# ChenFengTsai/dreamerv3-torch

Hardware: AMD Instinct MI355X
Metric: imagination-steps/sec (higher is better)
Workload: dtype f32; 1 GPU; cfg2: dmc_vision 64x64x3 synthetic replay, RSSM deter=512 hidden=512 stoch=32x32, continuous actor (6), imag_gradient dynamics, batch 16 x seq 64 per GPU, horizon 15; one step = full Dreamer._train update (world model + actor + critic fwd/bwd, gradient all-reduce, 3x clip+Adam); global_batch=16, seq_len=64, horizon=15, parallelism=dp1

## Files before the change

dreamerv3-torch_amd/csrc/fusedops.hip:

```cpp
#include "dv3_common.h"

namespace dv3 {

typedef float f32x4 __attribute__((ext_vector_type(4)));
typedef float f32x4u __attribute__((ext_vector_type(4), aligned(4)));

struct OLParams {
  const int* idx;
  int S, D;
  const float* x2;
  long ldx2;
  int A2;
  const float* WT;
  long ldw;
  const float* base;
  long ldbase;
  float* pre;
  long ldpre;
  const float* gamma;
  const float* beta;
  float* y;
  long ldy;
  float* mean;
  float* rstd;
  long M;
  int N;
  int act;
  const float* smp_logit;
  const float* smp_noise;
  const unsigned long long* smp_rng;
  unsigned long long smp_off;
  float* smp_onehot;
  int* smp_idx;
  const int* smp_forced;
  unsigned int* smp_flips;
  float smp_unimix;
  int smp_mode;
  const float* nb_first;
  const float* nb_init;
  const int* nb_init_idx;
  float* nb_out;
  int* nb_idx_out;
};

template <int NV4, bool SMP = false, bool RT = false>
__global__ __launch_bounds__(SMP ? 1024 : 256) void onehot_linear_ln_vec_kernel(OLParams p) {
  __shared__ __attribute__((aligned(16))) float part[4][256 * NV4];
  __shared__ int sidx[64];
  const int wave = threadIdx.x >> 6, l = threadIdx.x & 63;
  const float inv_n = 1.f / (float)p.N;
  constexpr int MAXB = 8;
  for (long r = blockIdx.x; r < p.M; r += gridDim.x) {
    int my;
    if constexpr (SMP) {
      const int d = threadIdx.x & 31;
      unsigned long long seed = 0, offset = 0;
      if (!p.smp_mode && !p.smp_noise) {
        seed = p.smp_rng[0];
        offset = p.smp_rng[1] + p.smp_off;
      }
      const float m = p.nb_first[r];
      __syncthreads();
      for (int sg = threadIdx.x >> 5; sg < p.S; sg += 32) {
        const long gi = r * p.S + sg;
        const float lg = p.smp_logit[gi * 32 + d];
        float sm, ph;
        unimix_probs<32>(lg, true, 32, p.smp_unimix, sm, ph);
        float score = ph;
        if (!p.smp_mode) {
          float q;
          if (p.smp_noise) {
            q = p.smp_noise[gi * 32 + d];
          } else {
            uint32_t o4[4];
            const unsigned long long e = (unsigned long long)gi * 32 + d;
            Philox ph4(seed);
            ph4(offset + (e >> 2), 0x5eedULL, o4);
            q = fmaxf(-logf(u01(o4[e & 3])), 1e-30f);
          }
          score = ph / q;
        }
        float best = score;
        int bi = d;
#pragma unroll
        for (int o = 16; o > 0; o >>= 1) {
          const float ob = __shfl_xor(best, o, 64);
          const int oi = __shfl_xor(bi, o, 64);
          if (ob > best || (ob == best && oi < bi)) {
            best = ob;
            bi = oi;
          }
        }
        if (p.smp_forced) {
          const int f = p.smp_forced[gi];
          if (d == 0 && p.smp_flips && f != bi) atomicAdd(p.smp_flips, 1u);
          bi = f;
        }
        const float v = (d == bi) ? 1.f : 0.f;
        p.smp_onehot[gi * 32 + d] = v;
        p.nb_out[gi * 32 + d] = v * (1.f - m) + p.nb_init[sg * 32 + d] * m;
        if (d == 0) {
          if (p.smp_idx) p.smp_idx[gi] = bi;
          const int ni = (m != 0.f) ? p.nb_init_idx[sg] : bi;
          p.nb_idx_out[gi] = ni;
          sidx[sg] = ni;
        }
      }
      __syncthreads();
      my = (l < p.S) ? sidx[l] : 0;
    } else {
      my = (l < p.S) ? p.idx[r * p.S + l] : 0;
    }
    const bool worker = !SMP || wave < 4;
    f32x4 acc[NV4];
#pragma unroll
    for (int v = 0; v < NV4; ++v) acc[v] = (f32x4){0.f, 0.f, 0.f, 0.f};
    if (worker) {
    if (wave == 0 && p.base) {
#pragma unroll
      for (int v = 0; v < NV4; ++v) acc[v] = *reinterpret_cast<const f32x4u*>(p.base + r * p.ldbase + 4 * (l + 64 * v));
    }
    for (int s0 = wave; s0 < p.S; s0 += 4 * MAXB) {
      f32x4 t[MAXB][NV4];
#pragma unroll
      for (int u = 0; u < MAXB; ++u) {
        const int s = s0 + 4 * u;
        if (s < p.S) {
          const int id = __builtin_amdgcn_readlane(my, s);
          const float* w = p.WT + (long)(s * p.D + id) * p.ldw + 4 * l;
#pragma unroll
          for (int v = 0; v < NV4; ++v) t[u][v] = *reinterpret_cast<const f32x4u*>(w + 256 * v);
        } else {
#pragma unroll
          for (int v = 0; v < NV4; ++v) t[u][v] = (f32x4){0.f, 0.f, 0.f, 0.f};
        }
      }
#pragma unroll
      for (int u = 0; u < MAXB; ++u)
#pragma unroll
        for (int v = 0; v < NV4; ++v) acc[v] += t[u][v];
    }
    for (int a = wave; a < p.A2; a += 4) {
      const float xa = p.x2[r * p.ldx2 + a];
      const float* w = p.WT + (long)(p.S * p.D + a) * p.ldw + 4 * l;
#pragma unroll
      for (int v = 0; v < NV4; ++v) acc[v] += xa * *reinterpret_cast<const f32x4u*>(w + 256 * v);
    }
    }
    __syncthreads();
    if (worker) {
#pragma unroll
      for (int v = 0; v < NV4; ++v) *reinterpret_cast<f32x4*>(&part[wave][4 * (l + 64 * v)]) = acc[v];
    }
    __syncthreads();
    if (!worker) continue;
#pragma unroll
    for (int v = 0; v < NV4; ++v) {
      const f32x4 a0 = *reinterpret_cast<const f32x4*>(&part[0][4 * (l + 64 * v)]);
      const f32x4 a1 = *reinterpret_cast<const f32x4*>(&part[1][4 * (l + 64 * v)]);
      const f32x4 a2 = *reinterpret_cast<const f32x4*>(&part[2][4 * (l + 64 * v)]);
      const f32x4 a3 = *reinterpret_cast<const f32x4*>(&part[3][4 * (l + 64 * v)]);
      acc[v] = (a0 + a1) + (a2 + a3);
      if ((v & 3) == wave) *reinterpret_cast<f32x4u*>(p.pre + r * p.ldpre + 4 * (l + 64 * v)) = acc[v];
    }
    if (!p.y) continue;
    float s = 0.f;
#pragma unroll
    for (int v = 0; v < NV4; ++v) s += (acc[v][0] + acc[v][1]) + (acc[v][2] + acc[v][3]);
    const float mean = group_sum<64>(s) * inv_n;
    float q = 0.f;
#pragma unroll
    for (int v = 0; v < NV4; ++v)
#pragma unroll
      for (int e = 0; e < 4; ++e) {
        const float d = acc[v][e] - mean;
        q += d * d;
      }
    const float rstd = rsqrtf(group_sum<64>(q) * inv_n + kLnEps);
#pragma unroll
    for (int v = 0; v < NV4; ++v) {
      if ((v & 3) != wave) continue;
      const f32x4 g = *reinterpret_cast<const f32x4u*>(p.gamma + 4 * (l + 64 * v));
      const f32x4 b = *reinterpret_cast<const f32x4u*>(p.beta + 4 * (l + 64 * v));
      f32x4 z;
#pragma unroll
      for (int e = 0; e < 4; ++e) {
        const float t = (acc[v][e] - mean) * rstd * g[e] + b[e];
        if constexpr (RT) z[e] = actf_(t, p.act);
        else z[e] = p.act ? siluf_(t) : t;
      }
      *reinterpret_cast<f32x4u*>(p.y + r * p.ldy + 4 * (l + 64 * v)) = z;
    }
    if (threadIdx.x == 0) {
      if (p.mean) p.mean[r] = mean;
      if (p.rstd) p.rstd[r] = rstd;
    }
  }
}

template <bool RT = false>
__global__ __launch_bounds__(256) void onehot_linear_ln_generic_kernel(OLParams p) {
  __shared__ float red[4];
  __shared__ int sidx[64];
  const int tid = threadIdx.x;
// ... 175 lines not shown
        } else {
          uint32_t o[4];
          Philox ph(seed);
          ph(offset + ((unsigned long long)e >> 2), 0x6e6f726dULL, o);
          const int j = (int)(e & 3);
          const float rad = sqrtf(-2.f * logf(u01(o[j & 2])));
          const float ang = 6.283185307179586f * u01(o[(j & 2) + 1]);
          eps = (j & 1) ? rad * sinf(ang) : rad * cosf(ang);
        }
        if (p.eps_out) p.eps_out[e] = eps;
        const float mu = tanhf(mr);
        const float sd = (p.max_std - p.min_std) * sigmoidf_(sr + 2.f) + p.min_std;
        const float pre = mu + sd * eps;
        p.action[e] = pre * (1.f / fmaxf(fabsf(pre), 1.f));
        en = 0.5f + 0.9189385332046727f + logf(sd);
      }
      en = group_sum<64>(en);
      if (l == 0 && p.ent) p.ent[r] = en;
    } else {
      const float m = group_max<64>(valid ? mr : -INFINITY);
      const float ex = valid ? expf(mr - m) : 0.f;
      const float sm = ex / group_sum<64>(ex);
      const float ph = valid ? sm * (1.f - p.unimix) + p.unimix / (float)p.A : 0.f;
      float qv = 1.f;
      if (valid) {
        if (p.noise) {
          qv = p.noise[e];
        } else {
          uint32_t o[4];
          Philox ph4(seed);
          ph4(offset + ((unsigned long long)e >> 2), 0x5eedULL, o);
          qv = fmaxf(-logf(u01(o[e & 3])), 1e-30f);
        }
      }
      float best = valid ? ph / qv : -INFINITY;
      int bi = l;
#pragma unroll
      for (int o = 32; o > 0; o >>= 1) {
        const float ob = __shfl_xor(best, o, 64);
        const int oi = __shfl_xor(bi, o, 64);
        if (ob > best || (ob == best && oi < bi)) {
          best = ob;
          bi = oi;
        }
      }
      if (p.forced) {
        const int f = p.forced[r];
        if (l == 0 && p.flips && f != bi) atomicAdd(p.flips, 1u);
        bi = f;
      }
      if (valid) p.action[e] = (l == bi) ? 1.f : 0.f;
      if (l == 0 && p.act_idx) p.act_idx[r] = bi;
      const float en = group_sum<64>(valid ? -ph * logf(ph) : 0.f);
      if (l == 0 && p.ent) p.ent[r] = en;
    }
  }
}

__global__ __launch_bounds__(256) void transpose2d_kernel(const float* __restrict__ src, long lds_, int R, int C,
                                                          float* __restrict__ dst, long ldd) {
  __shared__ float tile[32][33];
  const int tx = threadIdx.x & 31, ty = threadIdx.x >> 5;
  const int c0 = blockIdx.x * 32, r0 = blockIdx.y * 32;
#pragma unroll
  for (int j = 0; j < 32; j += 8) {
    const int r = r0 + ty + j, c = c0 + tx;
    tile[ty + j][tx] = (r < R && c < C) ? src[(long)r * lds_ + c] : 0.f;
  }
  __syncthreads();
#pragma unroll
  for (int j = 0; j < 32; j += 8) {
    const int c = c0 + ty + j, r = r0 + tx;
    if (c < C && r < R) dst[(long)c * ldd + r] = tile[tx][ty + j];
  }
}

constexpr int kTrJobs = 12;
struct TrJobs {
  const float* src[kTrJobs];
  float* dst[kTrJobs];
  long lds[kTrJobs], ldd[kTrJobs];
  int R[kTrJobs], C[kTrJobs], tiles_c[kTrJobs];
  int tile0[kTrJobs + 1];
  int n;
};
__global__ __launch_bounds__(256) void transpose2d_many_kernel(TrJobs jb) {
  __shared__ float tile[32][33];
  int k = 0;
  while (k + 1 < jb.n && (int)blockIdx.x >= jb.tile0[k + 1]) ++k;
  const int t = blockIdx.x - jb.tile0[k];
  const float* __restrict__ src = jb.src[k];
  float* __restrict__ dst = jb.dst[k];
  const long lds_ = jb.lds[k], ldd = jb.ldd[k];
  const int R = jb.R[k], C = jb.C[k];
  const int tx = threadIdx.x & 31, ty = threadIdx.x >> 5;
  const int c0 = (t % jb.tiles_c[k]) * 32, r0 = (t / jb.tiles_c[k]) * 32;
#pragma unroll
  for (int j = 0; j < 32; j += 8) {
    const int r = r0 + ty + j, c = c0 + tx;
    tile[ty + j][tx] = (r < R && c < C) ? src[(long)r * lds_ + c] : 0.f;
  }
  __syncthreads();
#pragma unroll
  for (int j = 0; j < 32; j += 8) {
    const int c = c0 + ty + j, r = r0 + tx;
    if (c < C && r < R) dst[(long)c * ldd + r] = tile[tx][ty + j];
  }
}

template <int G>
__global__ __launch_bounds__(256) void onehot_to_idx_kernel(const float* __restrict__ x, int* __restrict__ idx, long R,
                                                            int D) {
  constexpr int GPB = 256 / G;
  const int sub = threadIdx.x / G, d = threadIdx.x % G;
  for (long g0 = (long)blockIdx.x * GPB; g0 < R; g0 += (long)gridDim.x * GPB) {
    const long g = g0 + sub;
    float best = (g < R && d < D) ? x[g * D + d] : -INFINITY;
    int bi = d;
#pragma unroll
    for (int o = G / 2; o > 0; o >>= 1) {
      const float ob = __shfl_xor(best, o, 64);
      const int oi = __shfl_xor(bi, o, 64);
      if (ob > best || (ob == best && oi < bi)) {
        best = ob;
        bi = oi;
      }
    }
    if (g < R && d == 0) idx[g] = bi;
  }
}

static unsigned cap_grid(long n, long per_block, long cap) {
  long b = (n + per_block - 1) / per_block;
  if (b > cap) b = cap;
  if (b < 1) b = 1;
  return (unsigned)b;
}

}

using namespace dv3;

extern "C" int dv3_onehot_linear_ln_fwd(const int* idx, int S, int D, const float* x2, long ldx2, int A2,
                                        const float* WT, long ldw, const float* base, long ldbase, float* pre,
                                        long ldpre, const float* gamma, const float* beta, float* y, long ldy,
                                        float* mean, float* rstd, long M, int N, int act, void* stream) {
  if (M <= 0) return 0;
  if (!idx || !WT || !pre || S <= 0 || S > 64 || D <= 0 || N <= 0 || A2 < 0 || (A2 > 0 && !x2) || ldw < N ||
      ldpre < N || (base && ldbase < N) || !dv3_act_ok(act))
    return DV3_ERR_ARG;
  if (y && (!gamma || !beta || ldy < N)) return DV3_ERR_ARG;
  OLParams p{idx, S, D, x2, ldx2, A2, WT, ldw, base, ldbase, pre, ldpre, gamma, beta, y, ldy, mean, rstd, M, N, act};
  hipStream_t s = (hipStream_t)stream;
  const bool vec = (N % 256 == 0) && N <= 1024 && (ldw % 4 == 0) && (ldpre % 4 == 0) && (!base || ldbase % 4 == 0) &&
                   (!y || ldy % 4 == 0);
  if (vec) {
    const dim3 grid(cap_grid(M, 1, 32768)), block(256);
    if (dv3_act_rt(act)) switch (N / 256) {
      case 1: hipLaunchKernelGGL((onehot_linear_ln_vec_kernel<1, false, true>), grid, block, 0, s, p); break;
      case 2: hipLaunchKernelGGL((onehot_linear_ln_vec_kernel<2, false, true>), grid, block, 0, s, p); break;
      case 3: hipLaunchKernelGGL((onehot_linear_ln_vec_kernel<3, false, true>), grid, block, 0, s, p); break;
      default: hipLaunchKernelGGL((onehot_linear_ln_vec_kernel<4, false, true>), grid, block, 0, s, p); break;
    }
    else switch (N / 256) {
      case 1: hipLaunchKernelGGL((onehot_linear_ln_vec_kernel<1>), grid, block, 0, s, p); break;
      case 2: hipLaunchKernelGGL((onehot_linear_ln_vec_kernel<2>), grid, block, 0, s, p); break;
      case 3: hipLaunchKernelGGL((onehot_linear_ln_vec_kernel<3>), grid, block, 0, s, p); break;
      default: hipLaunchKernelGGL((onehot_linear_ln_vec_kernel<4>), grid, block, 0, s, p); break;
    }
  } else if (dv3_act_rt(act)) {
    hipLaunchKernelGGL(onehot_linear_ln_generic_kernel<true>, dim3(cap_grid(M, 1, 16384)), dim3(256), 0, s, p);
  } else {
    hipLaunchKernelGGL(onehot_linear_ln_generic_kernel<false>, dim3(cap_grid(M, 1, 16384)), dim3(256), 0, s, p);
  }
  return (int)hipGetLastError();
}

extern "C" int dv3_onehot_sample_linear_ln_fwd(const float* logit, const float* noise,
                                               const unsigned long long* rng_state, unsigned long long rng_offset,
                                               float* onehot, int* idx, const int* forced, unsigned int* flips,
                                               float unimix, int mode, const float* next_first, const float* init,
                                               const int* init_idx, float* next_out, int* next_idx, int S,
                                               const float* x2, long ldx2, int A2, const float* WT, long ldw,
                                               float* pre, long ldpre, const float* gamma, const float* beta, float* y,
                                               long ldy, float* mean, float* rstd, long M, int N, int act,
                                               void* stream) {
  if (M <= 0) return 0;
  if (!logit || !onehot || !next_first || !init || !init_idx || !next_out || !next_idx || !WT || !pre || !gamma ||
      !beta || !y || S <= 0 || S > 32 || N <= 0 || (N % 256) != 0 || N > 1024 || A2 < 0 || (A2 > 0 && !x2) ||
      ldw < N || ldpre < N || ldy < N || (ldw % 4) || (ldpre % 4) || (ldy % 4))
    return DV3_ERR_ARG;
  if (!dv3_act_ok(act) || dv3_act_rt(act)) return DV3_ERR_ARG;
  if (!mode && !noise && !rng_state) return DV3_ERR_ARG;
  OLParams p{nullptr, S, 32, x2, ldx2, A2, WT, ldw, nullptr, 0, pre, ldpre, gamma, beta, y, ldy, mean, rstd, M, N, act,
             logit, noise, rng_state, rng_offset, onehot, idx, forced, flips, unimix, mode, next_first, init, init_idx,
             next_out, next_idx};
  hipStream_t s = (hipStream_t)stream;
  const dim3 grid(cap_grid(M, 1, 32768)), block(1024);
  switch (N / 256) {
    case 1: hipLaunchKernelGGL((onehot_linear_ln_vec_kernel<1, true>), grid, block, 0, s, p); break;
    case 2: hipLaunchKernelGGL((onehot_linear_ln_vec_kernel<2, true>), grid, block, 0, s, p); break;
    case 3: hipLaunchKernelGGL((onehot_linear_ln_vec_kernel<3, true>), grid, block, 0, s, p); break;
    default: hipLaunchKernelGGL((onehot_linear_ln_vec_kernel<4, true>), grid, block, 0, s, p); break;
  }
  return (int)hipGetLastError();
}

extern "C" int dv3_actor_head_fwd_ex(const float* pre, long ldpre, const float* gamma, const float* beta, float* y,
                                     long ldy, float* mean, float* rstd, const float* Wm, const float* bm,
                                     const float* Ws, const float* bs, float* out_m, float* out_s, const float* noise,
                                     const unsigned long long* rng_state, unsigned long long rng_offset, float* eps_out,
                                     float* action, float* entropy, int* act_idx, const int* forced,
                                     unsigned int* flips, long M, int U, int A, float min_std, float max_std,
                                     float unimix, int onehot, int act, void* stream) {
  if (!dv3_act_ok(act)) return DV3_ERR_ARG;
  if (M <= 0) return 0;
  if (!pre || !gamma || !beta || !y || !Wm || !bm || !out_m || !action || U <= 0 || U > 1024 || A <= 0 || A > 64 ||
      ldpre < U || ldy < U)
    return DV3_ERR_ARG;
  if (!onehot && (!Ws || !bs || !out_s)) return DV3_ERR_ARG;
  if (onehot && Ws) return DV3_ERR_ARG;
  if (!noise && !rng_state) return DV3_ERR_ARG;
  AHParams p{pre, ldpre, gamma, beta, y, ldy, mean, rstd, Wm, bm, Ws, bs, out_m, out_s, noise, rng_state, rng_offset,
             eps_out, action, entropy, act_idx, forced, flips, M, U, A, min_std, max_std, unimix, onehot, act};
  hipStream_t s = (hipStream_t)stream;
  const dim3 grid(cap_grid(M, 4, 4096)), block(256);
  if (act != DV3_ACT_SILU) {
    if (U <= 64) hipLaunchKernelGGL((actor_head_kernel<1, true>), grid, block, 0, s, p);
    else if (U <= 256) hipLaunchKernelGGL((actor_head_kernel<4, true>), grid, block, 0, s, p);
    else if (U <= 512) hipLaunchKernelGGL((actor_head_kernel<8, true>), grid, block, 0, s, p);
    else hipLaunchKernelGGL((actor_head_kernel<16, true>), grid, block, 0, s, p);
    return (int)hipGetLastError();
  }
  if (U <= 64) hipLaunchKernelGGL((actor_head_kernel<1>), grid, block, 0, s, p);
  else if (U <= 256) hipLaunchKernelGGL((actor_head_kernel<4>), grid, block, 0, s, p);
  else if (U <= 512) hipLaunchKernelGGL((actor_head_kernel<8>), grid, block, 0, s, p);
  else hipLaunchKernelGGL((actor_head_kernel<16>), grid, block, 0, s, p);
  return (int)hipGetLastError();
}

extern "C" int dv3_actor_head_fwd(const float* pre, long ldpre, const float* gamma, const float* beta, float* y,
                                  long ldy, float* mean, float* rstd, const float* Wm, const float* bm,
                                  const float* Ws, const float* bs, float* out_m, float* out_s, const float* noise,
                                  const unsigned long long* rng_state, unsigned long long rng_offset, float* eps_out,
                                  float* action, float* entropy, int* act_idx, const int* forced,
                                  unsigned int* flips, long M, int U, int A, float min_std, float max_std,
                                  float unimix, int onehot, void* stream) {
  return dv3_actor_head_fwd_ex(pre, ldpre, gamma, beta, y, ldy, mean, rstd, Wm, bm, Ws, bs, out_m, out_s, noise, rng_state,
                               rng_offset, eps_out, action, entropy, act_idx, forced, flips, M, U, A, min_std, max_std,
                               unimix, onehot, DV3_ACT_SILU, stream);
}

extern "C" int dv3_transpose2d(const float* src, long lds, int R, int C, float* dst, long ldd, void* stream) {
  if (R <= 0 || C <= 0) return 0;
  if (!src || !dst || lds < C || ldd < R) return DV3_ERR_ARG;
  hipLaunchKernelGGL(transpose2d_kernel, dim3((C + 31) / 32, (R + 31) / 32), dim3(256), 0, (hipStream_t)stream, src,
                     lds, R, C, dst, ldd);
  return (int)hipGetLastError();
}

extern "C" int dv3_transpose2d_many(int njobs, const unsigned long long* jobs_host, void* stream) {
  if (njobs <= 0) return 0;
  if (!jobs_host || njobs > kTrJobs) return DV3_ERR_ARG;
  TrJobs jb;
  int tiles = 0;
  for (int k = 0; k < njobs; ++k) {
    const unsigned long long* j = jobs_host + 6 * k;
    jb.src[k] = (const float*)(uintptr_t)j[0];
    jb.dst[k] = (float*)(uintptr_t)j[1];
    jb.lds[k] = (long)j[2];
    jb.ldd[k] = (long)j[3];
    jb.R[k] = (int)j[4];
    jb.C[k] = (int)j[5];
    if (!jb.src[k] || !jb.dst[k] || jb.R[k] <= 0 || jb.C[k] <= 0 || jb.lds[k] < jb.C[k] || jb.ldd[k] < jb.R[k]) return DV3_ERR_ARG;
    jb.tiles_c[k] = (jb.C[k] + 31) / 32;
    jb.tile0[k] = tiles;
    tiles += jb.tiles_c[k] * ((jb.R[k] + 31) / 32);
  }
  for (int k = njobs; k <= kTrJobs; ++k) jb.tile0[k] = tiles;
  jb.n = njobs;
  hipLaunchKernelGGL(transpose2d_many_kernel, dim3((unsigned)tiles), dim3(256), 0, (hipStream_t)stream, jb);
  return (int)hipGetLastError();
}

extern "C" int dv3_onehot_to_idx(const float* onehot, int* idx, long R, int D, void* stream) {
  if (R <= 0) return 0;
  if (!onehot || !idx || D <= 0) return DV3_ERR_ARG;
  if (D > 64) return DV3_ERR_ARG;
  int G = 4;
  while (G < 64 && G < D) G <<= 1;
  hipStream_t s = (hipStream_t)stream;
  switch (G) {
    case 4: hipLaunchKernelGGL((onehot_to_idx_kernel<4>), dim3(cap_grid(R, 64, 8192)), dim3(256), 0, s, onehot, idx, R, D); break;
    case 8: hipLaunchKernelGGL((onehot_to_idx_kernel<8>), dim3(cap_grid(R, 32, 8192)), dim3(256), 0, s, onehot, idx, R, D); break;
    case 16: hipLaunchKernelGGL((onehot_to_idx_kernel<16>), dim3(cap_grid(R, 16, 8192)), dim3(256), 0, s, onehot, idx, R, D); break;
    case 32: hipLaunchKernelGGL((onehot_to_idx_kernel<32>), dim3(cap_grid(R, 8, 8192)), dim3(256), 0, s, onehot, idx, R, D); break;
    default: hipLaunchKernelGGL((onehot_to_idx_kernel<64>), dim3(cap_grid(R, 4, 8192)), dim3(256), 0, s, onehot, idx, R, D); break;
  }
  return (int)hipGetLastError();
}
```

dreamerv3-torch_amd/dv3hip/engine.py:

```python
from __future__ import annotations

from dataclasses import dataclass
from typing import Dict, List, Optional

import torch

from . import _dev, ops

F32 = torch.float32


_FUSE_BLEND = _dev.flag("DV3_FUSE_BLEND", True)
_FUSE_SAMPLE = _dev.flag("DV3_FUSE_SAMPLE", True)
_GATHER_OBS = _dev.flag("DV3_GATHER_OBS", True)
_FUSE_SAMPLE_IN = _dev.flag("DV3_FUSE_SAMPLE_IN", True)
_FUSE_CARRY = _dev.flag("DV3_FUSE_CARRY", True)
_FUSE_SCAN_ROW = _dev.flag("DV3_FUSE_SCAN_ROW", True)
_FUSE_SCAN_LN = _dev.flag("DV3_FUSE_SCAN_LN", True)
_FUSE_SCAN_LNBWD = _dev.flag("DV3_FUSE_SCAN_LNBWD", True)
_FUSE_SCAN_CS = _dev.flag("DV3_FUSE_SCAN_CS", True)
_DEFER_CONV_WGRAD = _dev.flag("DV3_DEFER_CONV_WGRAD", True)
_FUSE_SCAN_GRUBWD = _dev.flag("DV3_FUSE_SCAN_GRUBWD", True)
_ONEHOT_WGRAD = _dev.flag("DV3_ONEHOT_WGRAD", True)
_ONEHOT_WGRAD_MIN_WORK = 1 << 21
# ... 926 lines not shown
                               eps_out=bufs["eps"], mode=not sample, **self.head)
            return
        io = None if idx_out is None else idx_out.view(-1)
        if fuse_smp:
            ops.gemm_sample(bufs["x2"], P.ims.W, bufs["logit"].view(M, self.SD), bufs["stoch"], bias=P.ims.b,
                            noise=noise, rng=rng, idx=io, forced=forced, flips=flips, unimix=self.unimix,
                            mode=not sample)
        else:
            ops.gemm(bufs["x2"], P.ims.W, bufs["logit"].view(M, self.SD), bias=P.ims.b)
            ops.onehot_sample(bufs["logit"], bufs["stoch"], noise=noise, rng=rng, unimix=self.unimix, mode=not sample,
                              forced=forced, flips=flips, idx=io)

    def pack_bwd(self, defer=None):
        P, ws = self.P, self.ws
        wt = {"in": self.pack_img_in(defer=defer)}
        for nm, W in (("gru", P.gru.W), ("out", P.img_out.W), ("ims", P.ims.W)):
            t = ws.get(f"rssm.{nm}_wt", (W.shape[1], W.shape[0]))
            if defer is not None:
                defer.append((W, t))
            else:
                ops.transpose2d(W, t)
            wt[nm] = t
        return wt

    def img_step_bwd(self, dstoch, ddeter, prev_deter, bufs, scratch, dprev_stoch, dprev_deter, daction,
                     accumulate_prev=False, wt=None):
        P = self.P
        M = dstoch.shape[0]
        S, D, SD, De, Hd = self.S, self.D, self.SD, self.De, self.Hd
        dlogit = scratch["dlogit"]
        if self.gauss:
            ops.gauss_head_bwd(bufs["raw"], dlogit, dstoch=dstoch, eps=bufs["eps"], **self.head_bwd)
        else:
            ops.onehot_st_bwd(bufs["logit"], dstoch.view(M, S, D), dlogit.view(M, S, D), unimix=self.unimix)
        if wt is not None:
            ops.gemm(dlogit, wt["ims"], scratch["dx2"])
            dense_ln_bwd_pre(P.img_out, scratch["dx2"], bufs["x2pre"], bufs.get("m2"), bufs.get("r2"), scratch["dx2pre"],
                             wgrad=False)
            ops.gemm(scratch["dx2pre"], wt["out"], ddeter, accumulate=True)
            gru_gates_bwd(P.gru, ddeter, bufs["gpre"], prev_deter, bufs.get("mg"), bufs.get("rg"), scratch["dgpre"],
                          dprev_deter, wgrad=False, accumulate_dh=accumulate_prev)
            if M > 128 and ops.gemm_split_ok(scratch["dgpre"], wt["gru"]):
                ops.gemm_split(scratch["dgpre"], wt["gru"], scratch["dx1"], dprev_deter, accumulate2=True)
            else:
                ops.gemm(scratch["dgpre"], wt["gru"][Hd:], dprev_deter, accumulate=True)
                ops.gemm(scratch["dgpre"], wt["gru"][:Hd], scratch["dx1"])
            dense_ln_bwd_pre(P.img_in, scratch["dx1"], bufs["x1pre"], bufs.get("m1"), bufs.get("r1"), scratch["dx1pre"],
                             wgrad=False)
            if daction is not None and M > 128 and SD % 16 == 0 and ops.gemm_split_ok(scratch["dx1pre"], wt["in"]):
                ops.gemm_split(scratch["dx1pre"], wt["in"], dprev_stoch, daction, accumulate=accumulate_prev)
                return
            ops.gemm(scratch["dx1pre"], wt["in"][:SD], dprev_stoch, accumulate=accumulate_prev)
            if daction is not None:
                ops.gemm(scratch["dx1pre"], wt["in"][SD:], daction)
            return
        ops.gemm(dlogit, P.ims.W, scratch["dx2"], transB=False)
        dense_ln_bwd_pre(P.img_out, scratch["dx2"], bufs["x2pre"], bufs.get("m2"), bufs.get("r2"), scratch["dx2pre"],
                         wgrad=False)
        ops.gemm(scratch["dx2pre"], P.img_out.W, ddeter, transB=False, accumulate=True)
        gru_gates_bwd(P.gru, ddeter, bufs["gpre"], prev_deter, bufs.get("mg"), bufs.get("rg"), scratch["dgpre"],
                      dprev_deter, wgrad=False, accumulate_dh=accumulate_prev)
        ops.gemm(scratch["dgpre"], P.gru.W[:, Hd:], dprev_deter, transB=False, accumulate=True)
        ops.gemm(scratch["dgpre"], P.gru.W[:, :Hd], scratch["dx1"], transB=False)
        dense_ln_bwd_pre(P.img_in, scratch["dx1"], bufs["x1pre"], bufs.get("m1"), bufs.get("r1"), scratch["dx1pre"],
                         wgrad=False)
        ops.gemm(scratch["dx1pre"], P.img_in.W[:, :SD], dprev_stoch, transB=False, accumulate=accumulate_prev)
        if daction is not None:
            ops.gemm(scratch["dx1pre"], P.img_in.W[:, SD:], daction, transB=False)


@dataclass
class PConvLayer:
    W: torch.Tensor
    g: Optional[torch.Tensor] = None
    b: Optional[torch.Tensor] = None
    bias: Optional[torch.Tensor] = None
    act: int = 1
    out: bool = False

    def __post_init__(self):
        if self.bias is not None:
            self.out = True


_IM2COL_ROWS = _dev.value("DV3_IM2COL_ROWS", 2048)


class ConvEncoderEngine:
    def __init__(self, layers: List[PConvLayer], ws: Workspace, size=64):
        self.L, self.ws, self.size = layers, ws, size

    def forward(self, image_u8=None, perm=None, x_f32=None, keep=True):
        ws = self.ws
        H = self.size
        if x_f32 is not None:
            x, N = x_f32, x_f32.shape[0]
        else:
            N = image_u8.shape[0] * image_u8.shape[1]
            C = image_u8.shape[-1]
            x = ws.get("enc.x0", (N, H, H, C))
            ops.image_to_f32(image_u8, x, n_images=N, perm=perm)
        self._acts = []
        n_layers = len(self.L)
        for i, L in enumerate(self.L):
            Co, Ci = L.W.shape[0], L.W.shape[1]
            OH = H // 2
            pre = ws.get(f"enc.pre{i}", (N, OH, OH, Co))
            if N * OH * OH <= _IM2COL_ROWS and not keep:
                cols = ws.get(f"enc.cols{i}", (N * OH * OH, 16 * Ci))
                ops.im2col_s2(x, cols)
                ops.gemm(cols, L.W.view(Co, 16 * Ci), pre.view(N * OH * OH, Co))
            elif Ci == 3 and Co in ops.C3_WIDTHS:
                ops.conv_s2_c3_fwd(x, L.W, pre, CW=Co)
            else:
                wp = ws.get(f"enc.wp{i}", (Co, 16 * Ci))
                ops.pack_conv_weight(L.W, wp, transposed=False)
                ops.conv_s2_fwd(x, wp, pre, Ci=Ci, Co=Co)
            R = N * OH * OH
            mean, rstd = (ws.get(f"enc.m{i}", (R,)), ws.get(f"enc.r{i}", (R,))) if L.g is not None else (None, None)
            last = i == n_layers - 1
            y = ws.get(f"enc.y{i}", (N, Co * OH * OH) if last else (N, OH, OH, Co))
            ln_fwd(L, pre.view(R, Co), y if last else y.view(R, Co), mean, rstd, chw_group=OH * OH if last else 0)
            self._acts.append((x, pre, mean, rstd, y))
            x, H = y, OH
        return x

    def backward(self, dembed):
        ws = self.ws
        n_layers = len(self.L)
        dy = dembed
        for i in reversed(range(n_layers)):
            L = self.L[i]
            x, pre, mean, rstd, y = self._acts[i]
            Co, Ci = L.W.shape[0], L.W.shape[1]
            N, OH = pre.shape[0], pre.shape[1]
            R = N * OH * OH
            last = i == n_layers - 1
            dpre = ws.get(f"enc.dpre{i}", pre.shape)
            ln_bwd(L, dy if last else dy.view(R, Co), pre.view(R, Co), mean, rstd, dpre.view(R, Co), wgrad=True,
                   chw_group=OH * OH if last else 0)
            ops.conv_s2_wgrad(dpre, x, _g(L.W))
            if i > 0:
                wpt = ws.get(f"enc.wpt{i}", (4, Ci, 4 * Co))
                ops.pack_conv_weight(L.W, wpt, transposed=True)
                dx = ws.get(f"enc.dy{i - 1}", x.shape)
                ops.convT_s2_fwd(dpre, wpt, dx, Ci=Co, Co=Ci)
                dy = dx


class ConvDecoderEngine:
    def __init__(self, lin: PLin, layers: List[PConvLayer], ws: Workspace, minres=4):
        self.lin, self.L, self.ws, self.minres = lin, layers, ws, minres

    def forward(self, x1, x2):
        ws = self.ws
        R = x1.shape[0]
        E = self.lin.W.shape[0]
        mr = self.minres
        C0 = E // (mr * mr)
        h0 = ws.get("dec.h0", (R, mr, mr, C0))
        ops.gemm(x1, self.lin.W, h0.view(R, E), A2=x2, bias=self.lin.b)
        self._x = (x1, x2)
        self._acts = []
        x, H = h0, mr
        for i, L in enumerate(self.L):
            Ci, Co = L.W.shape[0], L.W.shape[1]
            OH = 2 * H
            c3 = L.out and Co == 3 and Ci in ops.C3_WIDTHS
            if not c3:
                wpt = ws.get(f"dec.wpt{i}", (4, Co, 4 * Ci))
                ops.pack_conv_weight(L.W, wpt, transposed=True)
            if not L.out:
                pre = ws.get(f"dec.pre{i}", (R, OH, OH, Co))
                ops.convT_s2_fwd(x, wpt, pre, Ci=Ci, Co=Co)
                rows = R * OH * OH
                mean, rstd = (ws.get(f"dec.m{i}", (rows,)), ws.get(f"dec.r{i}", (rows,))) if L.g is not None \
                    else (None, None)
                y = ws.get(f"dec.y{i}", (R, OH, OH, Co))
                ln_fwd(L, pre.view(rows, Co), y.view(rows, Co), mean, rstd)
                self._acts.append((x, pre, mean, rstd, y))
            else:
                y = ws.get("dec.recon", (R, OH, OH, Co))
                if c3:
                    ops.convT_s2_c3_fwd(x, L.W, y, CW=Ci, bias=L.bias, out_add=0.5)
                else:
                    ops.convT_s2_fwd(x, wpt, y, Ci=Ci, Co=Co, bias=L.bias, out_add=0.5)
                self._acts.append((x, None, None, None, y))
            x, H = y, OH
        return x

    def backward(self, drecon, dx1, dx2, *, acc_dx=False, defer=None, idx=None, D=0):
        ws = self.ws
        run = defer.append if defer is not None else (lambda f: f())
        dy = drecon
        for i in reversed(range(len(self.L))):
            L = self.L[i]
            x, pre, mean, rstd, y = self._acts[i]
            Ci, Co = L.W.shape[0], L.W.shape[1]
            R, OH = y.shape[0], y.shape[1]
            rows = R * OH * OH
            if not L.out:
                dpre = ws.get(f"dec.dpre{i}", pre.shape)
                ln_bwd(L, dy.view(rows, Co), pre.view(rows, Co), mean, rstd, dpre.view(rows, Co), wgrad=True)
            else:
                dpre = dy
                if L.bias is not None:
                    run(lambda dpre=dpre, L=L, rows=rows, Co=Co: ops.colsum(dpre.view(rows, Co), _g(L.bias),
                                                                         accumulate=True))
            (run if _DEFER_CONV_WGRAD else (lambda f: f()))(lambda x=x, dpre=dpre, L=L: ops.conv_s2_wgrad(x, dpre, _g(L.W)))
            dx = ws.get(f"dec.dx{i}", x.shape)
            if Co == 3 and Ci in ops.C3_WIDTHS:
                ops.conv_s2_c3_fwd(dpre, L.W, dx, CW=Ci)
            else:
                wp = ws.get(f"dec.wp{i}", (Ci, 16 * Co))
                ops.pack_conv_weight(L.W, wp, transposed=False)
                ops.conv_s2_fwd(dpre, wp, dx, Ci=Co, Co=Ci)
            dy = dx
        R = dy.shape[0]
        E = self.lin.W.shape[0]
        dh0 = dy.view(R, E)
        x1, x2 = self._x

        def _lin_wg():
            lin_wgrad_onehot(ws, "dec.lin", self.lin.W, dh0, idx, D, x1, x2)
            ops.colsum(dh0, _g(self.lin.b), accumulate=True)

        run(_lin_wg)
        k1 = x1.shape[1]
        ops.gemm(dh0, self.lin.W[:, :k1], dx1, transB=False, accumulate=acc_dx)
        ops.gemm(dh0, self.lin.W[:, k1:], dx2, transB=False, accumulate=acc_dx)


class EnsembleEngine:

    def __init__(self, name: str, bucket, layers: int, ws: Workspace, *, std: float, scale: float = 1.0, log: bool = True,
                 act=True):
        if bucket.members < 2 or layers < 1:
            raise ValueError("EnsembleEngine: needs at least 2 members (the unbiased std) and 1 trunk layer")
        self.name, self.bucket, self.L, self.ws = name, bucket, int(layers), ws
        self.K = bucket.members
        self.std, self.scale, self.log = float(std), float(scale), bool(log)
        self.act = ops.act_code(act)
        self._kept = None
        self._loss_ws = torch.zeros(ops.ENS_LOSS_WS, dtype=F32, device=ws.device)

    def _params(self):
        st = self.bucket.stacked
        layers = [(st(3 * i), st(3 * i + 1), st(3 * i + 2)) for i in range(self.L)]
        return layers, st(3 * self.L), st(3 * self.L + 1)

    def _acts(self, M: int, tag: str):
        layers, _, _ = self._params()
        ws, nm, K = self.ws, f"{self.name}.{tag}", self.K
        acts = []
        for i, ((W, _), _, _) in enumerate(layers):
            U = W.shape[1]
            acts.append((ws.get(f"{nm}.pre{i}", (K, M, U)), ws.get(f"{nm}.m{i}", (K * M,)),
                         ws.get(f"{nm}.r{i}", (K * M,)), ws.get(f"{nm}.y{i}", (K, M, U))))
        return acts

    def _trunk_fwd(self, x, tag: str):
        layers, _, _ = self._params()
        acts = self._acts(x.shape[0], tag)
        h = x
        for ((W, _), (g, _), (b, _)), (pre, mean, rstd, y) in zip(layers, acts):
            ops.ens_gemm(h, W, pre)
            ops.ens_ln_act_fwd(pre, g, b, y, mean, rstd, act=self.act)
            h = y
        return h, acts

    def _trunk_bwd(self, x, acts, dh, tag: str, *, wgrad: bool, dx=None, cols=None):
        layers, _, _ = self._params()
        ws, nm, K, M = self.ws, f"{self.name}.{tag}", self.K, x.shape[0]
        dy = dh
        for i in reversed(range(self.L)):
            (W, gW), (g, gg), (b, gb) = layers[i]
            pre, mean, rstd, _ = acts[i]
            dpre = ws.get(f"{nm}.dpre{i}", tuple(pre.shape))
            ops.ens_ln_act_bwd(dy, pre, g, b, mean, rstd, dpre, gg if wgrad else None, gb if wgrad else None,
                               act=self.act)
            if wgrad:
                ops.ens_gemm(dpre, acts[i - 1][3] if i > 0 else x, gW, transA=True, transB=False, accumulate=True)
            if i > 0:
                dprev = ws.get(f"{nm}.dy{i - 1}", tuple(acts[i - 1][3].shape))
                ops.ens_gemm(dpre, W, dprev, transB=False)
                dy = dprev
            elif dx is not None:
                ops.ens_gemm(dpre, W if cols is None else W[:, :, cols], dx, transB=False)

    def forward(self, x):
        _, (Wh, _), (bh, _) = self._params()
        M = x.shape[0]
        h, _ = self._trunk_fwd(x, f"f{M}")
        mu = self.ws.get(f"{self.name}.f{M}.mu", (self.K, M, Wh.shape[1]))
        ops.ens_gemm(h, Wh, mu, bias=bh)
        ops.tanh_fwd(mu, mu)
        return mu

    def regress_fwd_bwd(self, x, target):
        _, (Wh, gWh), (bh, gbh) = self._params()
        M, ws, nm = x.shape[0], self.ws, f"{self.name}.t{x.shape[0]}"
        h, acts = self._trunk_fwd(x, f"t{M}")
        pre = ws.get(f"{nm}.out", (self.K, M, Wh.shape[1]))
        ops.ens_gemm(h, Wh, pre, bias=bh)
        loss = ws.get(f"{nm}.loss", (1,))
        ops.ens_regress_loss(pre, target, pre, loss, self._loss_ws, self.std)
        ops.ens_gemm(pre, h, gWh, transA=True, transB=False, accumulate=True)
        ops.ens_colsum(pre, gbh, accumulate=True)
        dh = ws.get(f"{nm}.dh", tuple(h.shape))
        ops.ens_gemm(pre, Wh, dh, transB=False)
        self._trunk_bwd(x, acts, dh, f"t{M}", wgrad=True)
        return loss.view(())

    def disag_fwd(self, x, reward=None, *, keep: bool = True):
# ... 30 lines not shown
```

dreamerv3-torch_amd/models.py:

```python
from __future__ import annotations

import copy

import numpy as np
import torch
from torch import nn

import networks
import tools
from dv3hip import _dev
from dv3hip import engine as E
from dv3hip import ops
from dv3hip.params import ParamBucket

to_np = lambda x: x.detach().cpu().numpy()
_FUSED_IMAG = _dev.flag("DV3_FUSED_IMAG", True)
_STACK_DETER = _dev.flag("DV3_STACK_DETER", True)


import weakref

_BEHAVIORS = weakref.WeakKeyDictionary()
_RUNNERS = weakref.WeakKeyDictionary()

# ... 74 lines not shown
            self.dynamics = networks.RSSM(config.dyn_stoch, config.dyn_deter, config.dyn_hidden, config.dyn_rec_depth,
                                          config.dyn_discrete, config.act, config.norm, config.dyn_mean_act,
                                          config.dyn_std_act, config.dyn_min_std, config.unimix_ratio, config.initial,
                                          config.num_actions, self.embed_size, config.device)
            self.heads = nn.ModuleDict()
            feat_size = config.dyn_stoch * (config.dyn_discrete or 1) + config.dyn_deter
            self.heads["decoder"] = networks.MultiDecoder(feat_size, shapes, **config.decoder)
            self.heads["reward"] = networks.MLP(
                feat_size, (255,) if config.reward_head["dist"] == "symlog_disc" else (), config.reward_head["layers"],
                config.units, config.act, config.norm, dist=config.reward_head["dist"],
                outscale=config.reward_head["outscale"], device=config.device, name="Reward")
            self.heads["cont"] = networks.MLP(
                feat_size, (), config.cont_head["layers"], config.units, config.act, config.norm, dist="binary",
                outscale=config.cont_head["outscale"], device=config.device, name="Cont")
        if config.reward_head["dist"] != "symlog_disc":
            raise NotImplementedError("reward head: symlog_disc only")
        for name in config.grad_heads:
            assert name in self.heads, name
        self._model_opt = tools.Optimizer("model", list(self.parameters()), config.model_lr, config.opt_eps,
                                          config.grad_clip, config.weight_decay, opt=config.opt, use_amp=False)
        self._scales = dict(reward=config.reward_head["loss_scale"], cont=config.cont_head["loss_scale"])

    def preprocess(self, obs):
        dev = self._config.device
        obs = {k: torch.as_tensor(np.asarray(v) if not isinstance(v, torch.Tensor) else v).to(dev).to(torch.float32)
               for k, v in obs.items()}
        obs["image"] = obs["image"] / 255.0
        if "discount" in obs:
            obs["discount"] = (obs["discount"] * self._config.discount).unsqueeze(-1)
        assert "is_first" in obs and "is_terminal" in obs
        obs["cont"] = (1.0 - obs["is_terminal"]).unsqueeze(-1)
        return obs

    def _stage(self, data):
        dev = torch.device(self._config.device)
        out = {}
        for k, v in data.items():
            if isinstance(v, torch.Tensor):
                t = v.to(dev, non_blocking=True)
            else:
                t = torch.from_numpy(np.ascontiguousarray(v)).to(dev, non_blocking=True)
            if k == "image":
                if t.dtype != torch.uint8:
                    t = torch.clamp(torch.round(t.to(torch.float32)), 0, 255).to(torch.uint8)
                out[k] = t.contiguous()
            else:
                out[k] = t.to(torch.float32).contiguous()
        return out

    @tools.on_config_device
    def _train(self, data, noise=None):
        r = self._auto_runner() if noise is None else None
        if r is None:
            return self._train_eager(data, noise)
        return r.train_wm(data)

    def _auto_runner(self):
        r = _RUNNERS.get(self)
        if r is None:
            cfg = self._config
            beh = next((b() for b in _BEHAVIORS.get(self, []) if b() is not None), None)
            if (beh is None or not bool(getattr(cfg, "hip_graph", True)) or not torch.cuda.is_available()
                    or torch.device(cfg.device).type != "cuda"):
                return None
            from dv3hip.graph import UpdateRunner

            r = UpdateRunner(self, beh, use_graph=True)
            _RUNNERS[self] = r
        return r

    def _train_eager(self, data, noise=None):
        self.train_fwd_bwd(data, noise)
        return self.train_opt()

    def train_opt(self, allreduce=True):
        post, context, metrics, loss = self._pending
        metrics = dict(metrics)
        metrics.update(self._model_opt.finish(loss, allreduce))
        return post, context, _wrap(metrics)

    def train_fwd_bwd(self, data, noise=None):
        cfg = self._config
        st = self._stage(data)
        B, T = st["action"].shape[0], st["action"].shape[1]
        TB = B * T
        dev = st["action"].device
        dyn = self.dynamics
        rssm = dyn.engine
        ws = rssm.ws
        S, D, SD, De = dyn._stoch, dyn._discrete, dyn._stoch * (dyn._discrete or 1), dyn._deter
        gauss = not D
        nz = noise or {}
        rng = dyn._rng()
        self._model_opt.begin()

        act_tm = ops.transpose01(st["action"], ws.get("wm.action", (T, B, st["action"].shape[2])))
        first_tm = ops.transpose01(st["is_first"], ws.get("wm.first", (T, B)))
        reward_tm = ops.transpose01(st["reward"], ws.get("wm.reward", (T, B)))
        cont_tm = ws.get("wm.cont", (T, B))
        ops.transpose01(st["is_terminal"], cont_tm)
        ops.axpby(ws.get("wm.ones", (T, B)).fill_(1.0), cont_tm, 1.0, -1.0)

        enc = self.encoder
        cnn_eng = mlp_eng = None
        parts = []
        if enc.cnn_shapes:
            cnn_eng = enc._cnn.engine
            parts.append(cnn_eng.forward(st["image"], (B, T)))
        if enc.mlp_shapes:
            keys = list(enc.mlp_shapes)
            widths = [int(np.prod(enc.mlp_shapes[k])) for k in keys]
            xin = ws.get("wm.mlp_in", (TB, sum(widths)))
            raw = ws.get("wm.mlp_raw", (TB, sum(widths)))
            off = 0
            for k, w in zip(keys, widths):
                tmp = ops.transpose01(st[k].reshape(B, T, w), ws.get(f"wm.key.{k}", (T, B, w)))
                raw[:, off:off + w] = tmp.view(TB, w)
                off += w
            ops.symlog(raw, xin)
            mlp_eng = enc._mlp.engine_for(".wm")
            parts.append(mlp_eng.forward(xin)[0])
            self._enc_in = xin
        if len(parts) == 2:
            Ec, Em = parts[0].shape[1], parts[1].shape[1]
            embed = ws.get("wm.embed", (TB, Ec + Em))
            embed[:, :Ec].copy_(parts[0])
            embed[:, Ec:].copy_(parts[1])
        else:
            embed = parts[0]
        E_ = embed.shape[1]

        force = None
        if "force_post" in nz or "force_prior" in nz:
            force = dict(post=nz.get("force_post"), prior=nz.get("force_prior"), flips=nz.get("flips"))
        out = rssm.observe_fwd(embed.view(T, B, E_), act_tm, first_tm, q_prior=nz.get("q_prior"),
                               q_post=nz.get("q_post"), rng=rng, force=force)
        ps, dt = out["post_stoch"].view(TB, SD), out["deter"].view(TB, De)
        kl = ws.get("wm.kl", (T, B))
        ent_p, ent_q = ws.get("wm.ent_post", (T, B)), ws.get("wm.ent_prior", (T, B))
        if gauss:
            ops.gauss_kl_fwd(out["post_mean"], out["post_std"], out["prior_mean"], out["prior_std"], kl, ent_p, ent_q)
        else:
            ops.kl_fwd(out["post_logit"], out["prior_logit"], kl, ent_p, ent_q, unimix=dyn._unimix_ratio)
        lanes_pay = rssm.lanes_pay(heavy_side=bool(self.heads["decoder"].cnn_shapes))
        E.SideStream.host_sync_point(lanes_pay)

        up = 1.0 / TB
        dec = self.heads["decoder"]
        acc = ws.zeros("wm.acc", (8 + len(dec.mlp_shapes),))
        gs, gd = ws.get("wm.gs", (T, B, SD)), ws.get("wm.gd", (T, B, De))
        wrote = False
        deferred = []
        grad_heads = cfg.grad_heads
        if dec.cnn_shapes:
            dec_eng = dec._cnn.engine
            recon = dec_eng.forward(ps, dt)
            limg = ws.get("wm.loss_img", (TB,))
            drecon = ws.get("wm.drecon", recon.shape)
            ops.mse_image(recon, st["image"], limg, drecon, upstream=up, perm=(B, T))
            ops.dot_accumulate(limg, acc[1:2], scale=up)
            dec_eng.backward(drecon, gs.view(TB, SD), gd.view(TB, De), acc_dx=False, defer=deferred,
                             idx=out["post_idx"].view(TB, S) if E._GATHER_OBS and not gauss else None, D=D)
            self._defer_heads_from = len(deferred)
            wrote = True
            if "decoder" not in grad_heads:
                gs.zero_(), gd.zero_()
        if dec.mlp_shapes:
            mdec = dec._mlp
            deng = mdec.engine_for(".wm")
            h, _, _ = deng.forward(ps, dt)
            dh = ws.zeros("wm.dec_dh", h.shape)
            for ki, (k, shp) in enumerate(dec.mlp_shapes.items()):
                lin = mdec.mean_layer[k]
                w = int(np.prod(shp))
                mode = ws.get(f"wm.dec.{k}", (TB, w))
                ops.gemm(h, lin.weight, mode, bias=lin.bias)
                tgt = ops.transpose01(st[k].reshape(B, T, w), ws.get(f"wm.key.{k}", (T, B, w))).view(TB, w)
                lk = ws.get(f"wm.loss.{k}", (TB,))
                dmode = ws.get(f"wm.dmode.{k}", (TB, w))
                ops.symlog_mse(mode, tgt, lk, dmode, upstream=up)
                ops.dot_accumulate(lk, acc[8 + ki:9 + ki], scale=up)
                ops.gemm(dmode, lin.weight, dh, transB=False, accumulate=True)
                E.lin_wgrad(lin.weight, dmode, h)
                ops.colsum(dmode, lin.bias.grad, accumulate=True)
            gh = "decoder" in grad_heads
            deng.backward(ps, dt, slice(0, TB), wgrad=True, dh=dh, dx1=gs.view(TB, SD) if gh else None,
                          dx2=gd.view(TB, De) if gh else None, acc_dx=wrote, defer=deferred)
            wrote = wrote or gh
        if not wrote:
            gs.zero_(), gd.zero_()
        pidx = out["post_idx"].view(TB, S) if E._GATHER_OBS and not gauss else None
        reng = self.heads["reward"].engine_for(".wm")
        if pidx is not None:
            reng.pack_onehot(SD)
        _, r_logits, _ = reng.forward(ps, dt, idx=pidx, D=D)
        lp_r = ws.get("wm.lp_r", (TB,))
        ops.disc_logprob_fwd(r_logits, reward_tm.view(TB), lp_r)
        ops.dot_accumulate(lp_r, acc[2:3], scale=-up)
        dr = ws.get("wm.dr_logits", r_logits.shape)
        up_r = ws.get("wm.up_r", (TB,)).fill_(-up * self._scales["reward"])
        ops.disc_logprob_bwd(r_logits, reward_tm.view(TB), up_r, dr)
        g_r = "reward" in grad_heads
        reng.backward(ps, dt, slice(0, TB), dout=dr, wgrad=True, dx1=gs.view(TB, SD) if g_r else None,
                      dx2=gd.view(TB, De) if g_r else None, acc_dx=True, defer=deferred, idx=pidx, D=D)
        ceng = self.heads["cont"].engine_for(".wm")
        if pidx is not None:
            ceng.pack_onehot(SD)
        _, c_logit, _ = ceng.forward(ps, dt, idx=pidx, D=D)
        lp_c = ws.get("wm.lp_c", (TB,))
        ops.bernoulli_logprob_fwd(c_logit.view(TB), cont_tm.view(TB), lp_c)
        ops.dot_accumulate(lp_c, acc[3:4], scale=-up)
        dc = ws.get("wm.dc_logit", (TB, 1))
        up_c = ws.get("wm.up_c", (TB,)).fill_(-up * self._scales["cont"])
        ops.bernoulli_logprob_bwd(c_logit.view(TB), cont_tm.view(TB), up_c, dc.view(TB))
        g_c = "cont" in grad_heads
        ceng.backward(ps, dt, slice(0, TB), dout=dc, wgrad=True, dx1=gs.view(TB, SD) if g_c else None,
                      dx2=gd.view(TB, De) if g_c else None, acc_dx=True, defer=deferred, idx=pidx, D=D)
        if gauss:
            dpm, dps, dqm, dqs = (ws.get(f"wm.d{nm}", (T, B, S)) for nm in ("post_mean", "post_std", "prior_mean",
                                                                            "prior_std"))
            ops.gauss_kl_bwd(out["post_mean"], out["post_std"], out["prior_mean"], out["prior_std"], kl, dpost_mean=dpm,
                             dpost_std=dps, dprior_mean=dqm, dprior_std=dqs, free=cfg.kl_free, dyn_scale=cfg.dyn_scale,
                             rep_scale=cfg.rep_scale, upstream=up)
            dpl, dql = (dpm, dps), (dqm, dqs, None)
        else:
            dpl, dql = ws.get("wm.dpost_logit", (T, B, S, D)), ws.get("wm.dprior_logit", (T, B, S, D))
            ops.kl_bwd(out["post_logit"], out["prior_logit"], kl, dpl, dql, unimix=dyn._unimix_ratio, free=cfg.kl_free,
                       dyn_scale=cfg.dyn_scale, rep_scale=cfg.rep_scale, upstream=up)
        ops.dot_accumulate(kl.view(TB), acc[4:5], clip_min=cfg.kl_free, scale=up)
        dembed = ws.get("wm.dembed", (T, B, E_))
        side = rssm.observe_bwd(dpl, dql, gs, gd, dembed, extra_side=deferred, lanes_pay=lanes_pay)
        de = dembed.view(TB, E_)
        if cnn_eng is not None and mlp_eng is not None:
            Ec = parts[0].shape[1]
            d_cnn, d_mlp = ws.get("wm.dembed_cnn", (TB, Ec)), ws.get("wm.dembed_mlp", (TB, E_ - Ec))
            d_cnn.copy_(de[:, :Ec])
            d_mlp.copy_(de[:, Ec:])
        else:
            d_cnn = d_mlp = de
        with ops.gemm_group():
            if cnn_eng is not None:
                cnn_eng.backward(d_cnn)
            if mlp_eng is not None:
                mlp_eng.backward(self._enc_in, None, slice(0, TB), wgrad=True, dh=d_mlp)
        side.join()

        loss = ws.get("wm.loss", (1,))
        ops.dot_accumulate(kl.view(TB), ws.zeros("wm.kl_mean", (1,)), scale=up)
        ops.dot_accumulate(ent_q.view(TB), acc[5:6], scale=up)
        ops.dot_accumulate(ent_p.view(TB), acc[6:7], scale=up)
        loss.copy_(acc[1:2] + acc[8:].sum(0, keepdim=True) + self._scales["reward"] * acc[2:3]
                   + self._scales["cont"] * acc[3:4] + (cfg.dyn_scale + cfg.rep_scale) * acc[4:5])
        metrics = {}
        if dec.cnn_shapes:
            metrics["image_loss"] = acc[1]
        for ki, k in enumerate(dec.mlp_shapes):
            metrics[f"{k}_loss"] = acc[8 + ki]
        metrics.update(reward_loss=acc[2], cont_loss=acc[3], kl_free=cfg.kl_free, dyn_scale=cfg.dyn_scale,
                       rep_scale=cfg.rep_scale, dyn_loss=acc[4], rep_loss=acc[4], kl=ws.get("wm.kl_mean", (1,))[0],
                       prior_ent=acc[5], post_ent=acc[6])
        bt = lambda x: x.transpose(0, 1)
        post = dyn._state(out, "post", bt)
        self._last = dict(out=out, embed=embed.view(T, B, E_), kl=kl, ent_post=ent_p, action_tm=out["action"])
        context = _LazyContext(self, post)
        rng.commit()
        self._pending = (post, context, metrics, loss[0])

    @tools.on_config_device
    def video_pred(self, data, noise=None):
        data = self.preprocess(data)
        embed = self.encoder(data)
        nz = noise or {}
        states, _ = self.dynamics.observe(embed[:6, :5], data["action"][:6, :5], data["is_first"][:6, :5],
                                          noise=noise)
        recon = self.heads["decoder"](self.dynamics.get_feat(states))["image"].mode()[:6]
        init = {k: v[:, -1] for k, v in states.items()}
        prior = self.dynamics.imagine_with_action(data["action"][:6, 5:], init, noise=nz.get("q_open"))
        openl = self.heads["decoder"](self.dynamics.get_feat(prior))["image"].mode()
        model = torch.cat([recon[:, :5], openl], 1)
        truth = data["image"][:6]
        error = (model - truth + 1.0) / 2.0
        return torch.cat([truth, model, error], 2)


class _LazyContext(dict):

    def __init__(self, wm, post):
        super().__init__()
        self._wm, self._post = wm, post

    def __missing__(self, key):
        last = self._wm._last
        bt = lambda x: x.transpose(0, 1)
        if key == "embed":
            v = bt(last["embed"])
        elif key == "feat":
            v = self._wm.dynamics.get_feat(self._post)
        elif key == "kl":
            v = bt(last["kl"])
        elif key == "postent":
            v = bt(last["ent_post"])
        else:
            raise KeyError(key)
        self[key] = v
        return v


class EnsembleObjective:

    def __init__(self, engine, action_cond: bool, extr_scale: float):
        self.engine, self.action_cond, self.extr_scale = engine, bool(action_cond), float(extr_scale)


class ImagBehavior(nn.Module):
    def __init__(self, config, world_model, future_predictor=None):
        super().__init__()
        self._config = config
        self._world_model = world_model
        feat_size = config.dyn_stoch * (config.dyn_discrete or 1) + config.dyn_deter
        with _norm_scope(config):
            self.actor = networks.MLP(
                feat_size, (config.num_actions,), config.actor["layers"], config.units, config.act, config.norm,
                config.actor["dist"], config.actor["std"], config.actor["min_std"], config.actor["max_std"], absmax=1.0,
                temp=config.actor["temp"], unimix_ratio=config.actor["unimix_ratio"], outscale=config.actor["outscale"],
                name="Actor")
            self.value = networks.MLP(
                feat_size, (255,) if config.critic["dist"] == "symlog_disc" else (), config.critic["layers"], config.units,
                config.act, config.norm, config.critic["dist"], outscale=config.critic["outscale"], device=config.device,
                name="Value")
        _BEHAVIORS.setdefault(world_model, []).append(weakref.ref(self))
        if config.critic["dist"] != "symlog_disc" or config.actor["dist"] not in ("normal", "onehot"):
            raise NotImplementedError("critic symlog_disc; actor normal|onehot")
        if config.imag_gradient not in ("dynamics", "reinforce", "both"):
            raise NotImplementedError(config.imag_gradient)
        if config.critic["slow_target"]:
            self._slow_value = copy.deepcopy(self.value)
            self._updates = 0
        kw = dict(wd=config.weight_decay, opt=config.opt, use_amp=False)
        self._actor_opt = tools.Optimizer("actor", list(self.actor.parameters()), config.actor["lr"],
                                          config.actor["eps"], config.actor["grad_clip"], **kw)
        self._value_opt = tools.Optimizer("value", list(self.value.parameters()), config.critic["lr"],
                                          config.critic["eps"], config.critic["grad_clip"],
                                          extra=2 if config.reward_EMA else 0, **kw)
        if self._config.reward_EMA:
            self.register_buffer("ema_vals", torch.zeros((2,), device=self._config.device))
            self.reward_ema = RewardEMA(device=self._config.device)

    def _update_slow_target(self):
        if self._config.critic["slow_target"]:
            if self._updates % self._config.critic["slow_target_update"] == 0:
                mix = self._config.critic["slow_target_fraction"]
                vb = self._value_opt.bucket.ensure()
                sb = self._slow_bucket()
                ops.axpby(vb.flat, sb.flat, mix, 1.0 - mix)
            self._updates += 1

    def _slow_bucket(self):
        b = getattr(self, "_slow_b", None)
        if b is None:
            b = ParamBucket("slow_value", list(self._slow_value.parameters()))
# ... 445 lines not shown
```

Baseline: 1.233 million imagination-steps/s.

## Use one-hot gather for conv decoder input linear and batch weight transposes

The conv decoder's first linear layer now splits its input: the deterministic part goes through a normal GEMM, and the one-hot stochastic part becomes a row gather-add driven by the sampled indices instead of a dense GEMM over the 1024-wide one-hot vector. To handle the decoder's wide output (N > 1024), the one-hot linear kernel gains a column-sliced launch mode that uses blockIdx.y to offset into the weight and output. The transposes of the decoder, reward and cont weight slices are gathered up front into one batched transpose call, replacing separate launches. The aim is to cut FLOPs and kernel launches in the world-model forward, at the cost of an extra launch plus a read-modify-write of h0.

```diff
diff --git a/dreamerv3-torch_amd/csrc/fusedops.hip b/dreamerv3-torch_amd/csrc/fusedops.hip
--- a/dreamerv3-torch_amd/csrc/fusedops.hip
+++ b/dreamerv3-torch_amd/csrc/fusedops.hip
@@ -50,6 +50,12 @@
   const int wave = threadIdx.x >> 6, l = threadIdx.x & 63;
   const float inv_n = 1.f / (float)p.N;
   constexpr int MAXB = 8;
+  if constexpr (!SMP) {
+    const long c0 = (long)blockIdx.y * (256 * NV4);
+    p.WT += c0;
+    p.pre += c0;
+    if (p.base) p.base += c0;
+  }
   for (long r = blockIdx.x; r < p.M; r += gridDim.x) {
     int my;
     if constexpr (SMP) {
@@ -531,9 +537,19 @@
   if (y && (!gamma || !beta || ldy < N)) return DV3_ERR_ARG;
   OLParams p{idx, S, D, x2, ldx2, A2, WT, ldw, base, ldbase, pre, ldpre, gamma, beta, y, ldy, mean, rstd, M, N, act};
   hipStream_t s = (hipStream_t)stream;
-  const bool vec = (N % 256 == 0) && N <= 1024 && (ldw % 4 == 0) && (ldpre % 4 == 0) && (!base || ldbase % 4 == 0) &&
-                   (!y || ldy % 4 == 0);
-  if (vec) {
+  const bool al4 = (ldw % 4 == 0) && (ldpre % 4 == 0) && (!base || ldbase % 4 == 0) && (!y || ldy % 4 == 0);
+  const bool vec = (N % 256 == 0) && N <= 1024 && al4;
+  const bool sliced = !y && (N % 256 == 0) && N > 1024 && N / 256 <= 65535 && al4;
+  if (sliced) {
+    const int W = N % 1024 == 0 ? 1024 : N % 768 == 0 ? 768 : N % 512 == 0 ? 512 : 256;
+    const dim3 grid(cap_grid(M, 1, 32768), (unsigned)(N / W)), block(256);
+    switch (W / 256) {
+      case 1: hipLaunchKernelGGL((onehot_linear_ln_vec_kernel<1>), grid, block, 0, s, p); break;
+      case 2: hipLaunchKernelGGL((onehot_linear_ln_vec_kernel<2>), grid, block, 0, s, p); break;
+      case 3: hipLaunchKernelGGL((onehot_linear_ln_vec_kernel<3>), grid, block, 0, s, p); break;
+      default: hipLaunchKernelGGL((onehot_linear_ln_vec_kernel<4>), grid, block, 0, s, p); break;
+    }
+  } else if (vec) {
     const dim3 grid(cap_grid(M, 1, 32768)), block(256);
     if (dv3_act_rt(act)) switch (N / 256) {
       case 1: hipLaunchKernelGGL((onehot_linear_ln_vec_kernel<1, false, true>), grid, block, 0, s, p); break;
diff --git a/dreamerv3-torch_amd/dv3hip/engine.py b/dreamerv3-torch_amd/dv3hip/engine.py
--- a/dreamerv3-torch_amd/dv3hip/engine.py
+++ b/dreamerv3-torch_amd/dv3hip/engine.py
@@ -1102,14 +1102,32 @@
     def __init__(self, lin: PLin, layers: List[PConvLayer], ws: Workspace, minres=4):
         self.lin, self.L, self.ws, self.minres = lin, layers, ws, minres
 
-    def forward(self, x1, x2):
+    def gather_ok(self, SD: int) -> bool:
+        E, K = self.lin.W.shape
+        return _GATHER_OBS and E % 256 == 0 and 0 < SD < K
+
+    def pack_onehot(self, SD: int, defer=None):
+        W = self.lin.W
+        wt = self.ws.get("dec.lin_wt", (SD, W.shape[0]))
+        if defer is not None:
+            defer.append((W[:, :SD], wt))
+        else:
+            ops.transpose2d(W[:, :SD], wt)
+        return wt
+
+    def forward(self, x1, x2, *, idx=None, D=0):
         ws = self.ws
         R = x1.shape[0]
         E = self.lin.W.shape[0]
         mr = self.minres
         C0 = E // (mr * mr)
         h0 = ws.get("dec.h0", (R, mr, mr, C0))
-        ops.gemm(x1, self.lin.W, h0.view(R, E), A2=x2, bias=self.lin.b)
+        SD = 0 if idx is None else idx.shape[1] * D
+        if idx is not None and x2 is not None and x1.shape[1] == SD and self.gather_ok(SD):
+            ops.gemm(x2, self.lin.W[:, SD:], h0.view(R, E), bias=self.lin.b)
+            ops.onehot_linear_ln(idx, D, ws.get("dec.lin_wt", (SD, E)), h0.view(R, E), base=h0.view(R, E))
+        else:
+            ops.gemm(x1, self.lin.W, h0.view(R, E), A2=x2, bias=self.lin.b)
         self._x = (x1, x2)
         self._acts = []
         x, H = h0, mr
diff --git a/dreamerv3-torch_amd/models.py b/dreamerv3-torch_amd/models.py
--- a/dreamerv3-torch_amd/models.py
+++ b/dreamerv3-torch_amd/models.py
@@ -250,9 +250,21 @@
         wrote = False
         deferred = []
         grad_heads = cfg.grad_heads
+        pidx = out["post_idx"].view(TB, S) if E._GATHER_OBS and not gauss else None
+        reng = self.heads["reward"].engine_for(".wm")
+        ceng = self.heads["cont"].engine_for(".wm")
+        dec_idx = None
+        if pidx is not None:
+            tr = []
+            if dec.cnn_shapes and dec._cnn.engine.gather_ok(SD):
+                dec_idx = pidx
+                dec._cnn.engine.pack_onehot(SD, defer=tr)
+            reng.pack_onehot(SD, defer=tr)
+            ceng.pack_onehot(SD, defer=tr)
+            ops.transpose2d_many(tr)
         if dec.cnn_shapes:
             dec_eng = dec._cnn.engine
-            recon = dec_eng.forward(ps, dt)
+            recon = dec_eng.forward(ps, dt, idx=dec_idx, D=D)
             limg = ws.get("wm.loss_img", (TB,))
             drecon = ws.get("wm.drecon", recon.shape)
             ops.mse_image(recon, st["image"], limg, drecon, upstream=up, perm=(B, T))
@@ -287,10 +299,6 @@
             wrote = wrote or gh
         if not wrote:
             gs.zero_(), gd.zero_()
-        pidx = out["post_idx"].view(TB, S) if E._GATHER_OBS and not gauss else None
-        reng = self.heads["reward"].engine_for(".wm")
-        if pidx is not None:
-            reng.pack_onehot(SD)
         _, r_logits, _ = reng.forward(ps, dt, idx=pidx, D=D)
         lp_r = ws.get("wm.lp_r", (TB,))
         ops.disc_logprob_fwd(r_logits, reward_tm.view(TB), lp_r)
@@ -301,9 +309,6 @@
         g_r = "reward" in grad_heads
         reng.backward(ps, dt, slice(0, TB), dout=dr, wgrad=True, dx1=gs.view(TB, SD) if g_r else None,
                       dx2=gd.view(TB, De) if g_r else None, acc_dx=True, defer=deferred, idx=pidx, D=D)
-        ceng = self.heads["cont"].engine_for(".wm")
-        if pidx is not None:
-            ceng.pack_onehot(SD)
         _, c_logit, _ = ceng.forward(ps, dt, idx=pidx, D=D)
         lp_c = ws.get("wm.lp_c", (TB,))
         ops.bernoulli_logprob_fwd(c_logit.view(TB), cont_tm.view(TB), lp_c)
```

New measurement: 1.241 million imagination-steps/s (median of 6 runs). Within noise of the previous version (+0.7%).
